# Dxslab/mpi-petsc4py-example

Measured on AMD Instinct MI355X. Metric: CG iters/s + SpMV HBM GB/s (% peak), 3D Poisson 256³ at 1/2/4/8 GPUs, higher is better.
Workload: dtype f64

## Files before the change

mpi-petsc4py-example_amd/csrc/mx_abi.hip:

```cpp
#include <algorithm>
#include <atomic>
#include <cmath>
#include <cstdio>
#include <cstring>
#include <mutex>
#include <string>
#include <thread>
#include <vector>

#include "mx_internal.hpp"

struct mx_comm_s { mx::Comm *c; };
struct mx_mat_s { mx::Mat *A; };

namespace mx {

static thread_local std::string g_err;

[[noreturn]] void fail(int code, const std::string &msg) { throw Error(code, msg); }

void hip_check(hipError_t e, const char *what, const char *file, int line) {
  if (e != hipSuccess) {
    char buf[512];
    std::snprintf(buf, sizeof buf, "%s failed: %s (%s:%d)", what, hipGetErrorString(e), file, line);
// ... 550 lines not shown
  });
}
int mx_ksp_destroy(mx_mat a) {
  return guard([&] {
    Mat *A = M(a);
    (void)hipSetDevice(A->comm->device);
    HIPCHECK(hipStreamSynchronize(A->comm->stream));
    A->release_ksp();
  });
}
int mx_finalize(void) {
  return guard([&] {
    int nd = 0;
    if (hipGetDeviceCount(&nd) != hipSuccess) nd = 0;
    for (int d = 0; d < nd; ++d) {
      if (hipSetDevice(d) == hipSuccess) HIPCHECK(hipDeviceSynchronize());
    }
    (void)hipGetLastError();
    scratch_trim();
  });
}
int mx_vec_rhs_hash(mx_comm c, int64_t i0, int64_t n, double *b) {
  return guard([&] { Comm *k = C(c); vec_rhs_hash(k->stream, i0, n, b); HIPCHECK(hipStreamSynchronize(k->stream)); });
}

void mx_ksp_default_params(mx_ksp_params *p) {
  std::memset(p, 0, sizeof(*p));
  p->ksp_type = MX_KSP_GMRES;
  p->pc_type = MX_PC_JACOBI;
  p->norm_type = MX_NORM_DEFAULT;
  p->max_it = 10000;
  p->restart = 30;
  p->rtol = 1e-5;
  p->atol = 1e-50;
  p->dtol = 1e5;
  p->haptol = 1e-30;
  p->breakdowntol = 0.1;
  p->poll_every = 16;
}

int mx_lu_solve_csr(mx_comm c, int64_t n, const int64_t *indptr, const int64_t *cols,
                    const double *vals, const double *b, double *x) {
  return guard([&] { dense_lu_solve(C(c), n, indptr, cols, vals, b, x); });
}

int mx_dev_alloc(int device, size_t bytes, void **ptr) {
  return guard([&] {
    HIPCHECK(hipSetDevice(device));
    *ptr = nullptr;
    if (bytes && dev_malloc(ptr, bytes) != hipSuccess) { *ptr = nullptr; fail(MX_ERR_MEM, "device allocation failed"); }
  });
}

int mx_dev_free(void *ptr) { return guard([&] { dev_free(ptr); }); }

int mx_debug_set(int key, int value) {
  int old = -1;
  switch (key) {
    case 6: old = g_knobs.overlap; g_knobs.overlap = value; break;
    case 7: old = g_knobs.graph; g_knobs.graph = value; break;
    case 8: old = g_knobs.force_coll; g_knobs.force_coll = value; break;
    case 9: old = g_knobs.cg_fuse; g_knobs.cg_fuse = value; break;
    case 13: old = g_knobs.cg_vec; g_knobs.cg_vec = value; break;
    case 21: old = g_knobs.cg_unroll; g_knobs.cg_unroll = value; break;
    case 23: old = g_knobs.vcodes; g_knobs.vcodes = value; break;
    case 27: old = g_knobs.spmv_pairs; g_knobs.spmv_pairs = value; break;
    case 29: old = g_knobs.cg_xbatch; g_knobs.cg_xbatch = value; break;
    case 33: old = g_knobs.comm_timeout_ms; if (value > 0) g_knobs.comm_timeout_ms = value; break;
    case 38: old = g_knobs.pair_lean; g_knobs.pair_lean = value; break;
    case 39: old = g_knobs.pair_zm; g_knobs.pair_zm = value; break;
    case 40: old = g_knobs.pair_zm_bpc; g_knobs.pair_zm_bpc = std::min(std::max(value, 1), 8); break;
    case 41: old = g_knobs.pair_zm_len; g_knobs.pair_zm_len = std::min(std::max(value, 1), 1024); break;
    case 43: old = g_knobs.spmv_fp64_grid; g_knobs.spmv_fp64_grid = std::min(std::max(value, 0), 65536); break;
    case 47: old = g_knobs.comm_wait_ms; g_knobs.comm_wait_ms = std::max(value, 0); break;
    case 48: old = g_knobs.pair_col27; g_knobs.pair_col27 = value; break;
    case 52: old = g_knobs.pair_zmc; g_knobs.pair_zmc = value; break;
    case 53: old = g_knobs.pair_unitv; g_knobs.pair_unitv = value; break;
    case 60: old = g_knobs.pair_zm27p; g_knobs.pair_zm27p = value; break;
    case 70: old = g_knobs.zm27_2line; g_knobs.zm27_2line = value; break;
    case 72: old = g_knobs.asm_fused; g_knobs.asm_fused = value; break;
    case 80: old = g_knobs.cg_pbws; g_knobs.cg_pbws = value; break;
    case 81: old = g_knobs.scratch_cache; g_knobs.scratch_cache = value; if (!value) scratch_trim(); break;
    case 84: old = g_knobs.cb; g_knobs.cb = value; break;
    case 69: old = g_knobs.cg_pbw; g_knobs.cg_pbw = value; break;
    case 68: old = g_knobs.ru_2line; g_knobs.ru_2line = value; break;
    case 61: old = g_knobs.gm_stall_us; g_knobs.gm_stall_us = std::min(std::max(value, 0), 2000000); break;
    case 59: old = g_knobs.pw_sym27; g_knobs.pw_sym27 = value; break;
    default: break;
  }
  return old;
}

int mx_debug_assembly_times(double *out, int n) {
  const AsmTimes &t = g_asm_times;
  const double v[8] = {t.h2d_ms, t.canon_ms, t.split_ms, t.layout_ms, t.halo_ms, t.total_ms, t.host_bytes, t.alloc_ms};
  for (int k = 0; k < n && k < 8; ++k) out[k] = v[k];
  return 0;
}

int mx_debug_dispatch_counts(int64_t *out, int n, int reset) {
  for (int k = 0; k < DSP_COUNT; ++k) {
    const long long v = reset ? g_dispatch[k].exchange(0) : g_dispatch[k].load();
    if (out && k < n) out[k] = v;
  }
  return 0;
}

int mx_debug_stream_read(mx_comm c, const double *x, int64_t n, int width, double *out) {
  return guard([&] {
    Comm *k = C(c);
    debug_stream_read(k->stream, x, n, width, out);
    HIPCHECK(hipStreamSynchronize(k->stream));
  });
}

int mx_ksp_solve(mx_mat a, const mx_ksp_params *p, const double *b, double *x, mx_ksp_result *res,
                 double *history) {
  return guard([&] {
    Mat *A = M(a);
    ksp_solve(A, *p, b, x, *res, history);
  });
}

}

namespace mx {
void h2d_warm() {
  constexpr size_t W = (size_t)32 << 20;
  char *h = static_cast<char *>(std::aligned_alloc(4096, W));
  void *d = nullptr;
  hipStream_t st = nullptr;
  if (h && hipMalloc(&d, W) == hipSuccess && hipStreamCreateWithFlags(&st, hipStreamNonBlocking) == hipSuccess) {
    std::memset(h, 0, W);
    try {
      h2d_pinned({{d, h, W}}, st, (size_t)1 << 20);
    } catch (const Error &) {
    }
  }
  if (st) (void)hipStreamDestroy(st);
  if (d) (void)hipFree(d);
  std::free(h);
  (void)hipGetLastError();
}
}
```

mpi-petsc4py-example_amd/csrc/mx_internal.hpp:

```cpp
#pragma once

#include <hip/hip_runtime.h>

#include <atomic>
#include <cstdint>
#include <functional>
#include <memory>
#include <stdexcept>
#include <string>
#include <vector>

#include "mxsolve.h"

namespace mx {

struct Error : std::runtime_error {
  int code;
  Error(int c, const std::string &m) : std::runtime_error(m), code(c) {}
};

[[noreturn]] void fail(int code, const std::string &msg);
void hip_check(hipError_t e, const char *what, const char *file, int line);
#define HIPCHECK(x) ::mx::hip_check((x), #x, __FILE__, __LINE__)

// ... 78 lines not shown
  uint32_t lane[64];
};
struct PairUni27 {
  double v[54];
  unsigned long long pm[54];
  uint32_t flags, clean;
  uint32_t pad[2];
  unsigned long long lane[64];
};
constexpr uint32_t U27_ELO = 1u << 9;
constexpr uint32_t U27_EHI = 1u << 10;
constexpr uint32_t U27C_YLO = 1u << 0;
constexpr uint32_t U27C_YHI = 1u << 1;

struct Sell {
  int64_t nslices = 0, slots = 0, dia_slices = 0;
  int dia_k = 0;
  DBuf<int64_t> sptr;
  DBuf<int32_t> width;
  DBuf<int32_t> col;
  DBuf<double> val;
  DBuf<int32_t> doff;
  DBuf<int32_t> dpat;
  int64_t npat = 0;
  DBuf<uint32_t> mask;
  DBuf<uint8_t> mask8;
  int ntab = 0;
  int64_t code_bytes = 0;
  DBuf<uint8_t> code;
  DBuf<int64_t> cptr;
  DBuf<double> vtab;
  int32_t pat_star = -1;
  std::vector<int32_t> pat_star_off;
  std::vector<int32_t> pat_len;
  std::vector<int32_t> pat_host;
  int pair_shape = 0;
  int64_t nunits = 0;
  DBuf<uint8_t> pcode;
  DBuf<int32_t> pblk;
  int64_t pair_blocks = 0;
  int64_t pair_used = 0;
  bool pair_ghosts = false;
  bool pair_all = false;
  DBuf<PairUni> puni;
  bool pair_clean = false;
  DBuf<PairUni27> puni27;
  DBuf<double> pval;
  DBuf<int32_t> pflag;
  int pair_f64 = 0;
  bool pair_clean27 = false;
  bool pair_unit27 = false;
  bool pair_sym27 = false;
  bool pair_2l27 = false;
  bool pair_4l27 = false;
  DBuf<int32_t> pcol27;
  DBuf<double> dtab;
  bool pair_code_clean = false;
  int cb_bs = 0, cb_nblk = 0;
  DBuf<int64_t> cb_bstart;
  DBuf<int32_t> cb_col, cb_perm;
  DBuf<double> cb_val, cb_prod;
};
constexpr uint32_t PBLK_GHOST_LO = 1u << 30;
constexpr uint32_t PBLK_GHOST_HI = 1u << 31;
constexpr uint32_t PBLK_RUN0 = 1u << 22;
constexpr uint32_t PBLK_ELO = 1u << 27;
constexpr uint32_t PBLK_EHI = 1u << 28;
constexpr uint32_t PBLK_ID = PBLK_RUN0 - 1;
static_assert((PBLK_RUN0 << 4) < PBLK_ELO && PBLK_ELO < PBLK_EHI && PBLK_EHI < PBLK_GHOST_LO,
              "PBLK select-free flags overlap the ghost bits");
static_assert(((PBLK_RUN0 << 5) - PBLK_RUN0 | PBLK_ELO | PBLK_EHI | PBLK_ID) < PBLK_GHOST_LO, "PBLK field overlap");
constexpr int64_t PAIR_MAX_ROWS = int64_t(1) << 28;
constexpr int VCODE_MAX = 256;
constexpr int VCODE_ABSENT = VCODE_MAX - 1;
constexpr int CODE_BATCH = 8 * SLICE;
struct VCodes { const uint8_t *code; const int64_t *cptr; const double *tab; int ntab; };

struct Knobs {
  int overlap = 1; int graph = 1; int force_coll = 0; int cg_fuse = 3; int cg_vec = 0; int cg_unroll = 2;
  int vcodes = 1; int spmv_pairs = 1; int cg_xbatch = 0; int comm_timeout_ms = 120000;
  int pair_lean = 1; int pair_zm = 1; int pair_zm_bpc = 4; int pair_zm_len = 32; int spmv_fp64_grid = 8192;
  int comm_wait_ms = 600000; int pair_col27 = 1; int pair_zmc = 1; int pair_unitv = 1; int pw_sym27 = 1;
  int pair_zm27p = 1; int gm_stall_us = 0; int ru_2line = 3; int cg_pbw = 5; int zm27_2line = 1;
  int asm_fused = 1; int cg_pbws = 1; int scratch_cache = 1; int cb = 1;
  static constexpr int spmv_nt = 1, spmv_grid = 0, dia = 1, jac_const = 1, cg_fold = 1, ws_skew = 0;
  static constexpr int cg_vec_grid = 0, cg_nts = 0, bnd_grid = 0, mask8 = 1, cg_upd_grid = 0, spmv_ynt = 0;
  static constexpr int spmv_bpc = 6, spmv_pair_bpc = 4, pdict = 1, cg_ntl = 3, norm_grid = 0, pair_uni = 1;
  static constexpr int mdot_grid = 0, pair_dtab = 1, pair_zm_units = 2, pair_f64 = 1, pair_zm27_bpc = 6;
  static constexpr int cg5_fold = 1, pair_zm27_units = 1, gm_pad = 256, cg5_27 = 1, pair_zm27_ru_bpc = 5;
  static constexpr int pw_bpc = 0, ru_bpc = 3, zm_balance = 1, zm27_xcol = 1, zm27_xcol_ru = 2, zm27_xcol_pw = 3;
  static constexpr int maxpy_grid = 0, zmc_units = 1, zmc_bpc = 0;
};
extern Knobs g_knobs;

struct Halo {
  std::vector<int> recv_peer;
  std::vector<int64_t> recv_off, recv_cnt;
  std::vector<int> send_peer;
  std::vector<int64_t> send_off, send_cnt;
  std::vector<int64_t> send_contig_start;
  DBuf<int32_t> send_idx;
  DBuf<double> send_buf;
  DBuf<double> lvec;
  int64_t nsend = 0, nrecv = 0;
  bool need_pack = false;
  DBuf<int32_t> bnd_slices;
  int nbnd = 0;
  hipEvent_t ev_x = nullptr, ev_done = nullptr;
  ~Halo() {
    if (ev_x) (void)hipEventDestroy(ev_x);
    if (ev_done) (void)hipEventDestroy(ev_done);
  }
};

struct Mat {
  Comm *comm = nullptr;
  int64_t M = 0, N = 0, m = 0, n = 0, rstart = 0, cstart = 0, cend = 0;
  std::vector<int64_t> rranges, cranges;
  DBuf<int64_t> dptr, optr;
  DBuf<int32_t> dcol, ocol;
  DBuf<double> dval, oval, diag;
  DBuf<int64_t> garray;
  int64_t nnz_d = 0, nnz_o = 0, nghost = 0;
  std::vector<int64_t> garray_h;
  Sell sd, so;
  Halo halo;
  DBuf<double> partials;
  DBuf<double> scratch_x;
  DBuf<double> ksp_ws;
  DBuf<char> ksp_state;
  DBuf<double> jac_dinv;
  int jac_mode = -1;
  double jac_c = 1.0;
  int sym = -1;
  hipGraphExec_t cg_graph = nullptr;
  std::vector<uintptr_t> cg_key;
  bool cg_graph_failed = false;
  int *poll_pinned = nullptr;
  void *state_pinned = nullptr;
  hipEvent_t poll_ev[2] = {nullptr, nullptr};
  hipEvent_t solve_ev[2] = {nullptr, nullptr};
  void release_ksp();
  ~Mat() { release_ksp(); }
};

struct AsmTimes {
  double h2d_ms = 0, canon_ms = 0, split_ms = 0, layout_ms = 0, halo_ms = 0, total_ms = 0;
  double alloc_ms = 0;
  double host_bytes = 0;
};
extern thread_local AsmTimes g_asm_times;
double wall_ms();

struct AssemblyInput {
  const int64_t *rowptr = nullptr;
  const int64_t *coo_rows = nullptr;
  const int64_t *cols = nullptr;
  const int32_t *cols32 = nullptr;
  const double *vals = nullptr;
  int64_t nnz = 0;
  int insert_mode = MX_INSERT_VALUES;
};
Mat *assemble(Comm *c, int64_t M, int64_t N, int64_t m_local, int64_t n_local,
              const AssemblyInput &in);
void stencil_coo(Comm *c, int kind, int64_t nx, int64_t ny, int64_t nz, int64_t row0,
                 int64_t m, DBuf<int64_t> &rows, DBuf<int64_t> &cols, DBuf<int32_t> &cols32,
                 DBuf<double> &vals);
void convert_index(const void *src, int bytes, int64_t n, int64_t *dst, hipStream_t s);

struct Jac {
  const double *d = nullptr;
  double c = 1.0;
  int mode = 0;
};
__device__ __forceinline__ double papply(const Jac &J, double r, int64_t i) {
  return J.mode == 1 ? r * J.d[i] : (J.mode == 2 ? r * J.c : r);
}

enum SpmvMode { SPMV_PLAIN = 0, SPMV_JACOBI = 1, SPMV_DOT = 2, SPMV_CG = 3,
                SPMV_PLAIN_S = 4, SPMV_JACOBI_S = 5,
                SPMV_PW = 6, SPMV_RUPD = 7 };
constexpr bool spmv_jac(int mode) { return mode == SPMV_JACOBI || mode == SPMV_JACOBI_S; }
constexpr bool spmv_scaled(int mode) { return mode == SPMV_PLAIN_S || mode == SPMV_JACOBI_S; }
struct KspState;
struct Fold;
struct CgFuse {
  const double *r = nullptr;
  const double *pold = nullptr;
  double *pnew = nullptr;
  double *x = nullptr;
  KspState *st = nullptr;
  double *hist = nullptr;
  Jac jac;
};
void halo_begin(Mat *A, const double *x);
void spmv_launch(Mat *A, const double *x, double *y, int mode, Jac jac, double *partials,
                 int *done_flag);
int matmult_overlap(Mat *A, const double *x, double *y, int mode, Jac jac, double *partials,
                    int *done_flag, const CgFuse *cg = nullptr, const Fold *fold = nullptr,
                    const double *xscale = nullptr);
int spmv_blocks(const Mat *A, int mode = SPMV_PLAIN);
struct ExtTiming { hipEvent_t a = nullptr, b = nullptr; bool armed = false, used = false; };
extern thread_local ExtTiming g_ext_timing;
enum Dispatch {
  DSP_SELL = 0,
  DSP_SELL_CG = 1,
  DSP_PAIR_LEAN = 2,
  DSP_PAIR_ZM = 3,
  DSP_PAIR_ZM_SPLIT = 4,
  DSP_PAIR_ZM27 = 5,
  DSP_PAIR_ZM27_SPLIT = 6,
  DSP_PAIR_ZMF64 = 7,
  DSP_PAIR_ZMF64_SPLIT = 8,
  DSP_PAIR_ZMCG = 9,
  DSP_BOUNDARY = 10,
  DSP_ZM_PW = 11,
  DSP_ZM_RUPD = 12,
  DSP_PAIR_ZMC = 13,
  DSP_PAIR_ZMC_SPLIT = 14,
  DSP_ZM_PBW = 15,
  DSP_ZM_PBWS = 16,
  DSP_CB = 17,
  DSP_COUNT = 18
};
void note_dispatch(int kind);
extern std::atomic<long long> g_dispatch[DSP_COUNT];
int device_cu_count();
int main_grid(const Mat *A, int mode, const void *kf, bool pairs);
int pair_lean_launch(Mat *A, int mode, bool split, const double *x, double *y, double *partials, const int *done,
                     const Fold &fold, hipStream_t st, const Jac &jac = Jac{}, const double *xscale = nullptr);
bool pair_code_applies(const Mat *A);
void pair_sym_prepare(Mat *A);
int pair_lean_kind(const Mat *A);
bool pair_zm_applies(const Mat *A);
int pair_f64_kind(const Mat *A);
bool pair_cg5_applies(const Mat *A, int jac_mode);
int pair_cg5_rupd_launch(Mat *A, KspState *s, const double *p, const double *w, double *r, const double *r0,
                         int jac_mode, double jac_c, double *partials, const Fold &fold, const double *dot_part,
                         int ndot, int xb, int *hw, hipStream_t st);
bool pair_cg5_pbw_applies(const Mat *A, int jac_mode, int xb);
int pair_cg5_pbw_launch(Mat *A, KspState *s, const double *r, const double *r0, double *const pb[8], int xb,
                        double *hist, int jac_mode, double jac_c, double *partials, const Fold &fold,
                        hipStream_t st);
bool pair_cg5_pbws_applies(const Mat *A, int jac_mode, int xb);
int pair_cg5_pbws_launch(Mat *A, KspState *s, const double *r, double *const pb[8], int xb, double *hist, int jac_mode,
                         double jac_c, double *y, double *partials, hipStream_t st);
int cg5_pbws_matmult(Mat *A, KspState *s, const double *r, double *const pb[8], int xb, int it, double *hist,
                     const Jac &jac, double *y, double *partials, int *done, const Fold *fold);
bool matmult_splits(const Mat *A);
void mat_mult(Mat *A, const double *x, double *y);
void build_cb(Mat *A, hipStream_t st);
bool cb_applies(const Mat *A, int mode, bool split);
int cb_launch(Mat *A, int mode, bool split, const double *x, double *y, const Jac &jac, double *partials,
              const int *done, const Fold &fold, const double *xscale, hipStream_t st);

constexpr int RED_BLOCKS = 1024;
void finish_reduce(const double *partials, int nblocks, int nvals, double *out, hipStream_t s,
                   int *done_flag = nullptr);
double host_dot(Comm *c, int64_t n, const double *x, const double *y);
void host_mdot(Comm *c, int64_t n, const double *x, int nv, const double *const *y, double *out_host);
void vec_maxpy(hipStream_t s, int64_t n, double *y, int nv, const double *alpha, const double *const *x);
void vec_axpy(hipStream_t s, int64_t n, double a, const double *x, double *y);
void vec_aypx(hipStream_t s, int64_t n, double a, const double *x, double *y);
void vec_pmult(hipStream_t s, int64_t n, const double *x, const double *y, double *w);
void vec_scale(hipStream_t s, int64_t n, double a, double *x);
void vec_set(hipStream_t s, int64_t n, double a, double *x);
void vec_rhs_hash(hipStream_t s, int64_t i0, int64_t n, double *b);
void debug_stall(hipStream_t s, int stall_us);
void flush_read(hipStream_t s, const double *x, int64_t n, double *partials);
void debug_stream_read(hipStream_t s, const double *x, int64_t n, int width, double *out);
void exclusive_scan_i64(const int64_t *in, int64_t *out, int64_t n, hipStream_t s,
                        int64_t *total_host);

void dense_lu_solve(Comm *c, int64_t n, const int64_t *ip, const int64_t *cj, const double *vv,
                    const double *b, double *x);

void ksp_solve(Mat *A, const mx_ksp_params &p, const double *b, double *x, mx_ksp_result &r,
               double *hist);

inline int64_t cdiv(int64_t a, int64_t b) { return (a + b - 1) / b; }
inline unsigned grid_for(int64_t n, int block, int64_t cap = 1 << 16) {
  int64_t g = cdiv(n, block);
  if (g < 1) g = 1;
  if (g > cap) g = cap;
  return (unsigned)g;
}

void load_code_comm();
void load_code_vec();
void load_code_assembly();
void load_code_spmv();
void load_code_spmv_pair();
void load_code_spmv_cb();
void load_code_ksp();
void load_code_direct();
void load_code_objects();
void h2d_warm();

}
```

mpi-petsc4py-example_amd/csrc/mx_spmv_pair.hip:

```cpp
#include "mx_cg.hpp"
#include "mx_device.hpp"
#include "mx_internal.hpp"
#include "mx_pair.hpp"
#include "mx_launch.hpp"

namespace mx {

constexpr int PAIR_OOR = 1 << 28;
constexpr int PAIR_OOR_EDGE = 1 << 27;
constexpr int64_t PAIR_CLEAN_MAX_ROWS = int64_t(1) << 27;
constexpr int LEAN_WAVES = 4;

struct PairLeanArgs {
  int m, n, nunits;
  int anchor[5];
  int P, NZ, L, S;
  double *partials;
  const int *done;
  Fold fold;
};

template <int PS, bool CLEAN>
__device__ __forceinline__ dbl2 pair_sums(const dbl2 (&L)[PairShape<PS>::NR], double e, uint32_t bw,
                                          const PairUni *__restrict__ puni, int lane) {
// ... 280 lines not shown
  int sb, se, W, w;
  if ((gridDim.x & 7) == 0) {
    const int xcd = blockIdx.x & 7;
    W = (gridDim.x >> 3) * LEAN_WAVES;
    w = (blockIdx.x >> 3) * LEAN_WAVES + wid;
    sb = a.S * xcd / 8;
    se = a.S * (xcd + 1) / 8;
  } else {
    W = gridDim.x * LEAN_WAVES;
    w = blockIdx.x * LEAN_WAVES + wid;
    sb = 0;
    se = a.S;
  }
  const __amdgpu_buffer_rsrc_t xr = vec_rsrc(x, a.n);
  const int D = a.anchor[LAST], NL = a.anchor[3];
  const int PL = NL / 128, PH = a.P / 2;
  const int ecst = lane == 0 ? a.anchor[TR] - 1 : 128 + a.anchor[TR];
  constexpr uint32_t CARRY = PBLK_RUN0 | (PBLK_RUN0 << TR) | (PBLK_RUN0 << LAST);
  double nv[3] = {0.0, 0.0, 0.0};
  const int ntask = (se - sb) * PH;
  for (int t = w; t < ntask; t += W) {
    const int seg = sb + t / PH, cp = t % PH;
    const int colA = (cp / PL) * 2 * PL + cp % PL, colB = colA + PL;
    const int z0 = seg * a.L, z1 = min(z0 + a.L, a.NZ);
    const int cbA = colA * 128 + 2 * lane, cbB = colB * 128 + 2 * lane;
    dbl2 zmA = bload2(xr, z0 * D + cbA - D), cA = bload2(xr, z0 * D + cbA);
    dbl2 zmB = bload2(xr, z0 * D + cbB - D), cB = bload2(xr, z0 * D + cbB);
    uint32_t bwAn = (uint32_t)pblk[z0 * a.P + colA], bwBn = (uint32_t)pblk[z0 * a.P + colB];
    for (int z = z0; z < z1; ++z) {
      const uint32_t bwA = bwAn, bwB = bwBn;
      if (z + 1 < z1) { bwAn = (uint32_t)pblk[(z + 1) * a.P + colA]; bwBn = (uint32_t)pblk[(z + 1) * a.P + colB]; }
      const int rA = z * D + cbA, rB = z * D + cbB;
      const dbl2 zpA = bload2(xr, rA + D), zpB = bload2(xr, rB + D);
      const dbl2 nA = bload2(xr, rA + a.anchor[1] + ((bwA & (PBLK_RUN0 << 1)) ? PAIR_OOR : 0));
      const dbl2 nB = bload2(xr, rB + a.anchor[3] + ((bwB & (PBLK_RUN0 << 3)) ? PAIR_OOR : 0));
      int eA = ecst, eB = ecst;
      eA += lane == 0 ? ((bwA & PBLK_ELO) ? PAIR_OOR : 0) : ((bwA & PBLK_EHI) ? PAIR_OOR : 0);
      eB += lane == 0 ? ((bwB & PBLK_ELO) ? PAIR_OOR : 0) : ((bwB & PBLK_EHI) ? PAIR_OOR : 0);
      const double edA = bload1(xr, z * D + colA * 128 + eA), edB = bload1(xr, z * D + colB * 128 + eB);
      const dbl2 rqA = __builtin_nontemporal_load(reinterpret_cast<const dbl2 *>(rin + rA));
      const dbl2 rqB = __builtin_nontemporal_load(reinterpret_cast<const dbl2 *>(rin + rB));
      __builtin_amdgcn_sched_barrier(0);
      const dbl2 Z{0.0, 0.0};
      dbl2 LA[NR] = {zmA, nA, cA, (bwA & (PBLK_RUN0 << 3)) ? Z : cB, zpA};
      dbl2 LB[NR] = {zmB, (bwB & (PBLK_RUN0 << 1)) ? Z : cA, cB, nB, zpB};
      if (bwA & CARRY) {
        if (bwA & PBLK_RUN0) LA[0] = Z;
        if (bwA & (PBLK_RUN0 << TR)) LA[TR] = Z;
        if (bwA & (PBLK_RUN0 << LAST)) LA[LAST] = Z;
      }
      if (bwB & CARRY) {
        if (bwB & PBLK_RUN0) LB[0] = Z;
        if (bwB & (PBLK_RUN0 << TR)) LB[TR] = Z;
        if (bwB & (PBLK_RUN0 << LAST)) LB[LAST] = Z;
      }
      const dbl2 wA = pair_sums<PS, true>(LA, edA, bwA, puni, lane);
      const dbl2 wB = pair_sums<PS, true>(LB, edB, bwB, puni, lane);
      auto upd = [&](dbl2 w2, dbl2 rq, int r0) __attribute__((always_inline)) {
        const double ra = fma(-alpha, w2.x, rq.x), rb = fma(-alpha, w2.y, rq.y);
        const double za = JM == 2 ? ra * ru.c : ra, zb = JM == 2 ? rb * ru.c : rb;
        nv[0] += za * za; nv[1] += za * ra; nv[2] += ra * ra;
        nv[0] += zb * zb; nv[1] += zb * rb; nv[2] += rb * rb;
        *reinterpret_cast<dbl2 *>(ru.r + r0) = dbl2{ra, rb};
      };
      upd(wA, rqA, rA);
      upd(wB, rqB, rB);
      zmA = cA; cA = zpA;
      zmB = cB; cB = zpB;
    }
  }
  block_partials<3>(nv, a.partials, gridDim.x, a.fold);
}

struct PairPbArgs {
  KspState *s;
  const double *r;
  const double *r0;
  double *pb;
  int64_t ps;
  double *hist;
  double c;
};

template <int PS, int JM, int B, int ZU>
__global__ void __launch_bounds__(256) spmv_pair_pbw_kernel(const PairLeanArgs a, const int32_t *__restrict__ pblk,
                                                            const PairUni *__restrict__ puni, const PairPbArgs pa) {
  KspState *s = pa.s;
  const CgTopIn top = s->top;
  if (top.done) return;
  const CgTop t = cg_top(top);
  if (blockIdx.x == 0 && threadIdx.x == 0) cg_commit_top(s, t, pa.hist);
  if (t.reason) return;
  const int i = t.i;
  const double b = t.b;
  using SH = PairShape<PS>;
  constexpr int NR = SH::NR, TR = PS == 5 ? 1 : 2, LAST = NR - 1, C = SH::CENTER_RUN;
  auto pick = [&](int k) -> double * { return pa.pb + k * pa.ps; };
  double *pout = pick(i % B);
  const double *pprev = pick((i + B - 1) % B);
  const double *rs = (pa.r0 && i == 0) ? pa.r0 : pa.r;
  const int lane = threadIdx.x & 63;
  const int wid = __builtin_amdgcn_readfirstlane(threadIdx.x >> 6);
  int sb, se, W, w;
  if ((gridDim.x & 7) == 0) {
    const int xcd = blockIdx.x & 7;
    W = (gridDim.x >> 3) * LEAN_WAVES;
    w = (blockIdx.x >> 3) * LEAN_WAVES + wid;
    sb = a.S * xcd / 8;
    se = a.S * (xcd + 1) / 8;
  } else {
    W = gridDim.x * LEAN_WAVES;
    w = blockIdx.x * LEAN_WAVES + wid;
    sb = 0;
    se = a.S;
  }
  const __amdgpu_buffer_rsrc_t rr = vec_rsrc(rs, a.n), pr = vec_rsrc(pprev, a.n);
  const int D = a.anchor[LAST];
  const int eoff = 128 + a.anchor[TR];
  constexpr uint32_t CARRY = PBLK_RUN0 | (PBLK_RUN0 << TR) | (PBLK_RUN0 << LAST);
  const int ntask = (se - sb) * a.P;
  double dot = 0.0;
  auto march = [&](auto npc) __attribute__((always_inline)) {
    constexpr bool NP = decltype(npc)::value;
    auto dir = [&](dbl2 r2, dbl2 p2) __attribute__((always_inline)) {
      return dbl2{cg_dir(jac1<JM>(r2.x, 0.0, pa.c), b, NP ? 0.0 : p2.x),
                  cg_dir(jac1<JM>(r2.y, 0.0, pa.c), b, NP ? 0.0 : p2.y)};
    };
    for (int tk = w; tk < ntask; tk += W) {
      const int seg = sb + tk / a.P, col = tk % a.P;
      const int z0 = seg * a.L, z1 = min(z0 + a.L, a.NZ);
      const int cb = col * 128 + 2 * lane;
      dbl2 pc = dir(bload2(rr, z0 * D + cb), NP ? dbl2{0.0, 0.0} : bload2(pr, z0 * D + cb));
      uint32_t bwn = (uint32_t)pblk[z0 * a.P + col];
      auto step = [&](int z, auto nq) __attribute__((always_inline)) {
        constexpr int NQ = decltype(nq)::value;
        dbl2 zr[NQ], zpp[NQ], nr[NQ], npp[NQ];
        double er[NQ], epp[NQ];
        uint32_t bw[NQ];
        bw[0] = bwn;
#pragma unroll
        for (int q = 1; q < NQ; ++q) bw[q] = (uint32_t)pblk[(z + q) * a.P + col];
        if (z + NQ < z1) bwn = (uint32_t)pblk[(z + NQ) * a.P + col];
#pragma unroll
        for (int q = 0; q < NQ; ++q) {
          const int r0 = (z + q) * D + cb, ub = (z + q) * D + col * 128;
          zr[q] = bload2(rr, r0 + D);
          zpp[q] = NP ? dbl2{0.0, 0.0} : bload2(pr, r0 + D);
          if constexpr (PS == 7) {
            const int no = r0 + a.anchor[3] + ((bw[q] & (PBLK_RUN0 << 3)) ? PAIR_OOR : 0);
            nr[q] = bload2(rr, no);
            npp[q] = NP ? dbl2{0.0, 0.0} : bload2(pr, no);
          }
          er[q] = 0.0;
          epp[q] = 0.0;
          if (!(bw[q] & PBLK_EHI)) {
            er[q] = bload1(rr, ub + eoff);
            if constexpr (!NP) epp[q] = bload1(pr, ub + eoff);
          }
        }
        __builtin_amdgcn_sched_barrier(0);
#pragma unroll
        for (int q = 0; q < NQ; ++q) {
          const int r0 = (z + q) * D + cb;
          const dbl2 pz = dir(zr[q], zpp[q]);
          const double pe = cg_dir(jac1<JM>(er[q], 0.0, pa.c), b, NP ? 0.0 : epp[q]);
          *reinterpret_cast<dbl2 *>(pout + r0) = pc;
          dbl2 L[NR];
          L[0] = dbl2{0.0, 0.0};
          if constexpr (PS == 7) { L[1] = dbl2{0.0, 0.0}; L[3] = dir(nr[q], npp[q]); }
          L[TR] = pc;
          L[LAST] = pz;
          if (bw[q] & CARRY) {
            if (bw[q] & (PBLK_RUN0 << TR)) L[TR] = dbl2{0.0, 0.0};
            if (bw[q] & (PBLK_RUN0 << LAST)) L[LAST] = dbl2{0.0, 0.0};
          }
          const dbl2 tq = pair_fwd<PS>(L, pe, bw[q], puni);
          dot += L[C].x * tq.x;
          dot += L[C].y * tq.y;
          pc = pz;
        }
      };
      int z = z0;
      for (; z + ZU <= z1; z += ZU) step(z, std::integral_constant<int, ZU>{});
      for (; z < z1; ++z) step(z, std::integral_constant<int, 1>{});
    }
  };
  const std::true_type T{};
  const std::false_type F{};
  if (b == 0.0) march(T);
  else march(F);
  double v[1] = {dot};
  block_partials<1>(v, a.partials, gridDim.x, a.fold);
}

template <int PS, bool CLEAN, int ZU, int JM>
__global__ void __launch_bounds__(256) spmv_pair_zmpbs_kernel(const PairLeanArgs a, double *__restrict__ y,
                                                              const int32_t *__restrict__ pblk,
                                                              const PairUni *__restrict__ puni, const PairPbArgs pa,
                                                              int xb) {
  KspState *s = pa.s;
  const CgTopIn top = s->top;
  if (top.done) return;
  const CgTop t = cg_top(top);
  if (blockIdx.x == 0 && threadIdx.x == 0) cg_commit_top(s, t, pa.hist);
  if (t.reason) return;
  const int i = t.i;
  const double b = t.b;
  double *pout = pa.pb + (int64_t)(i % xb) * pa.ps;
  const double *pprev = pa.pb + (int64_t)((i + xb - 1) % xb) * pa.ps;
  using SH = PairShape<PS>;
  constexpr int NR = SH::NR, TR = PS == 5 ? 1 : 2, LAST = NR - 1;
  const int lane = threadIdx.x & 63;
  const int wid = __builtin_amdgcn_readfirstlane(threadIdx.x >> 6);
  int sb, se, W, w;
  if ((gridDim.x & 7) == 0) {
    const int xcd = blockIdx.x & 7;
    W = (gridDim.x >> 3) * LEAN_WAVES;
    w = (blockIdx.x >> 3) * LEAN_WAVES + wid;
    sb = a.S * xcd / 8;
    se = a.S * (xcd + 1) / 8;
  } else {
    W = gridDim.x * LEAN_WAVES;
    w = blockIdx.x * LEAN_WAVES + wid;
    sb = 0;
    se = a.S;
  }
  const __amdgpu_buffer_rsrc_t rr = vec_rsrc(pa.r, a.n), pr = vec_rsrc(pprev, a.n);
  const int D = a.anchor[LAST];
  const int ecst = lane == 0 ? a.anchor[TR] - 1 : 128 + a.anchor[TR];
  constexpr uint32_t CARRY = PBLK_RUN0 | (PBLK_RUN0 << TR) | (PBLK_RUN0 << LAST);
  auto dir1 = [&](double r1, double p1) __attribute__((always_inline)) {
    return cg_dir(jac1<JM>(r1, 0.0, pa.c), b, p1);
  };
  auto dir2 = [&](dbl2 r2, dbl2 p2) __attribute__((always_inline)) { return dbl2{dir1(r2.x, p2.x), dir1(r2.y, p2.y)}; };
  auto ld2 = [&](int off) __attribute__((always_inline)) { return dir2(bload2(rr, off), bload2(pr, off)); };
  double dot = 0.0;
  const int ntask = (se - sb) * a.P;
  for (int tk = w; tk < ntask; tk += W) {
    const int seg = sb + tk / a.P, col = tk % a.P;
    const int z0 = seg * a.L, z1 = min(z0 + a.L, a.NZ);
    const int cb = col * 128 + 2 * lane;
    dbl2 zm = ld2(z0 * D + cb - D), c = ld2(z0 * D + cb);
    uint32_t bwn = (uint32_t)pblk[z0 * a.P + col];
    auto step = [&](int z, auto nq) __attribute__((always_inline)) {
      constexpr int NQ = decltype(nq)::value;
      dbl2 L[NQ][NR], zp[NQ], zr[NQ], zq[NQ], Lr[NQ][NR], Lp[NQ][NR];
      double e[NQ], er[NQ], ep[NQ];
      uint32_t bw[NQ];
      bw[0] = bwn;
#pragma unroll
      for (int q = 1; q < NQ; ++q) bw[q] = (uint32_t)pblk[(z + q) * a.P + col];
      if (z + NQ < z1) bwn = (uint32_t)pblk[(z + NQ) * a.P + col];
#pragma unroll
      for (int q = 0; q < NQ; ++q) {
        const int r0 = (z + q) * D + cb, ub = (z + q) * D + col * 128;
        zr[q] = bload2(rr, r0 + D);
        zq[q] = bload2(pr, r0 + D);
#pragma unroll
        for (int r = 1; r < LAST; ++r)
          if (r != TR) {
            const int off = r0 + a.anchor[r] + (CLEAN && (bw[q] & (PBLK_RUN0 << r)) ? PAIR_OOR : 0);
            Lr[q][r] = bload2(rr, off);
            Lp[q][r] = bload2(pr, off);
          }
        int eo = ecst;
        if constexpr (CLEAN) eo += lane == 0 ? ((bw[q] & PBLK_ELO) ? PAIR_OOR : 0) : ((bw[q] & PBLK_EHI) ? PAIR_OOR : 0);
        er[q] = bload1(rr, ub + eo);
        ep[q] = bload1(pr, ub + eo);
      }
      __builtin_amdgcn_sched_barrier(0);
#pragma unroll
      for (int q = 0; q < NQ; ++q) {
// ... 1262 lines not shown
  if (pair_code_applies(A) && (split || (A->nghost == 0 && !S.pair_ghosts)))
    return pair_code_launch(A, mode, split, x, y, partials, done, fold_in, jac, xscale, st);
  if (xscale) return 0;
  if (mode != SPMV_PLAIN && mode != SPMV_DOT && mode != SPMV_PW) return 0;
  if (mode == SPMV_PW && !pair_cg5_applies(A, 0)) return 0;
  if (pair_f64_kind(A) && (split || A->nghost == 0))
    return pair_f64_launch(A, mode, split, x, y, partials, done, fold_in, st);
  const int kind = pair_lean_kind(A);
  if (!kind) return 0;
  if (!split && (A->nghost > 0 || S.pair_ghosts)) return 0;
  const bool clean = kind == 2;
  if (S.pair_shape == 27) return zm27_launch(A, mode, split, clean, x, y, partials, done, fold_in, st, PairRuArgs{}, 0);
  PairLeanArgs a{};
  a.m = (int)A->m;
  a.n = (int)A->n;
  a.nunits = (int)S.nunits;
  pair_anchors(S, a.anchor);
  a.partials = partials;
  a.done = done;
  const int NR = S.pair_shape == 5 ? 3 : 5, D = a.anchor[NR - 1];
  const bool zm = pair_zm_applies(A);
  LeanFn f = nullptr;
  ZmFn fz = nullptr;
  int grid;
  if (zm) {
    a.P = D / 128;
    a.NZ = (int)(A->m / D);
    grid = zm_tasks(a.P, a.NZ, a.L, a.S, mode == SPMV_PW && g_knobs.pw_bpc > 0 ? g_knobs.pw_bpc : g_knobs.pair_zm_bpc);
#define ZM_PICK(MODE, PS, SP, CL) \
    fz = g_knobs.pair_zm_units == 2 ? &spmv_pair_zm_kernel<MODE, PS, SP, CL, 2> : &spmv_pair_zm_kernel<MODE, PS, SP, CL, 1>
#define ZM_C(MODE, PS) do { if (split) { if (clean) ZM_PICK(MODE, PS, true, true); else ZM_PICK(MODE, PS, true, false); } \
                            else { if (clean) ZM_PICK(MODE, PS, false, true); else ZM_PICK(MODE, PS, false, false); } } while (0)
    if (mode == SPMV_PLAIN) { if (S.pair_shape == 5) ZM_C(SPMV_PLAIN, 5); else ZM_C(SPMV_PLAIN, 7); }
    else if (mode == SPMV_PW && clean && !split && A->sym == 1 && g_knobs.pw_sym27) {
      if (S.pair_shape == 5) fz = g_knobs.pair_zm_units == 2 ? &spmv_pair_zm_kernel<SPMV_PW, 5, false, true, 2, 0, true>
                                                             : &spmv_pair_zm_kernel<SPMV_PW, 5, false, true, 1, 0, true>;
      else fz = g_knobs.pair_zm_units == 2 ? &spmv_pair_zm_kernel<SPMV_PW, 7, false, true, 2, 0, true>
                                           : &spmv_pair_zm_kernel<SPMV_PW, 7, false, true, 1, 0, true>;
    }
    else if (mode == SPMV_PW) { if (S.pair_shape == 5) ZM_C(SPMV_PW, 5); else ZM_C(SPMV_PW, 7); }
    else { if (S.pair_shape == 5) ZM_C(SPMV_DOT, 5); else ZM_C(SPMV_DOT, 7); }
#undef ZM_C
#undef ZM_PICK
  } else {
#define LEAN_C(MODE, PS) do { if (split) f = clean ? &spmv_pair_lean_kernel<MODE, PS, true, true> : &spmv_pair_lean_kernel<MODE, PS, true, false>; \
                              else f = clean ? &spmv_pair_lean_kernel<MODE, PS, false, true> : &spmv_pair_lean_kernel<MODE, PS, false, false>; } while (0)
    if (mode == SPMV_PLAIN) { if (S.pair_shape == 5) LEAN_C(SPMV_PLAIN, 5); else LEAN_C(SPMV_PLAIN, 7); }
    else { if (S.pair_shape == 5) LEAN_C(SPMV_DOT, 5); else LEAN_C(SPMV_DOT, 7); }
#undef LEAN_C
    grid = main_grid(A, mode, reinterpret_cast<const void *>(f), true);
  }
  Fold fold = fold_in;
  if (fold.cnt) { fold.ntotal = fold.ncount = grid; fold.base = 0; }
  a.fold = fold;
  note_dispatch(mode == SPMV_PW ? DSP_ZM_PW : !zm ? DSP_PAIR_LEAN : split ? DSP_PAIR_ZM_SPLIT : DSP_PAIR_ZM);
  if (zm) launch_timed(fz, grid, st, a, x, y, S.pblk.p, S.puni.p, PairRuArgs{});
  else launch_timed(f, grid, st, a, x, y, S.pblk.p, S.puni.p);
  HIPCHECK(hipGetLastError());
  return grid;
}

bool pair_cg5_applies(const Mat *A, int jac_mode) {
  if (jac_mode != 0 && jac_mode != 2) return false;
  if (A->sd.pair_shape == 27)
    return g_knobs.cg5_27 && pair_lean_kind(A) == 2 && A->sd.pcol27.p && A->nghost == 0 && !A->sd.pair_ghosts;
  return pair_lean_kind(A) > 0 && pair_zm_applies(A) && ((A->nghost == 0 && !A->sd.pair_ghosts) || matmult_splits(A));
}

static int cg5_args(const Mat *A, PairLeanArgs &a, int bpc = 0) {
  const Sell &S = A->sd;
  a = PairLeanArgs{};
  a.m = (int)A->m;
  a.n = (int)A->n;
  a.nunits = (int)S.nunits;
  pair_anchors(S, a.anchor);
  const int D = a.anchor[S.pair_shape == 5 ? 2 : 4];
  a.P = D / 128;
  a.NZ = (int)(A->m / D);
  return zm_tasks(a.P, a.NZ, a.L, a.S, bpc);
}

bool pair_cg5_pbw_applies(const Mat *A, int jac_mode, int xb) {
  const int on = g_knobs.cg_pbw != 5 ? g_knobs.cg_pbw
                                     : A->m <= (int64_t(1) << (A->sd.pair_shape == 5 ? 24 : 23));
  return on && (xb == 2 || xb == 4 || xb == 8) && (jac_mode == 0 || jac_mode == 2) && pair_cg5_applies(A, jac_mode) &&
         A->sd.pair_shape != 27 && pair_lean_kind(A) == 2 && A->nghost == 0 && !A->sd.pair_ghosts && A->sym == 1 &&
         g_knobs.pw_sym27 && pair_zm_applies(A);
}

int pair_cg5_pbw_launch(Mat *A, KspState *s, const double *r, const double *r0, double *const pb[8], int xb,
                        double *hist, int jac_mode, double jac_c, double *partials, const Fold &fold_in,
                        hipStream_t st) {
  if (!pair_cg5_pbw_applies(A, jac_mode, xb)) return 0;
  const Sell &S = A->sd;
  PairLeanArgs a{};
  a.m = (int)A->m;
  a.n = (int)A->n;
  a.nunits = (int)S.nunits;
  pair_anchors(S, a.anchor);
  a.partials = partials;
  const int NR = S.pair_shape == 5 ? 3 : 5, D = a.anchor[NR - 1];
  a.P = D / 128;
  a.NZ = (int)(A->m / D);
  const int grid = zm_tasks(a.P, a.NZ, a.L, a.S, g_knobs.pw_bpc > 0 ? g_knobs.pw_bpc : g_knobs.pair_zm_bpc);
  Fold fold = fold_in;
  if (fold.cnt) { fold.ntotal = fold.ncount = grid; fold.base = 0; }
  a.fold = fold;
  const PairPbArgs pa{s, r, r0, pb[0], pb[1] - pb[0], hist, jac_c};
  using PbwFn = void (*)(const PairLeanArgs, const int32_t *, const PairUni *, const PairPbArgs);
  PbwFn f;
  const bool z2 = g_knobs.pair_zm_units == 2;
#define PBW(PS, JM, B) f = z2 ? &spmv_pair_pbw_kernel<PS, JM, B, 2> : &spmv_pair_pbw_kernel<PS, JM, B, 1>
#define PBW_B(PS, JM) do { if (xb == 8) PBW(PS, JM, 8); else if (xb == 4) PBW(PS, JM, 4); else PBW(PS, JM, 2); } while (0)
#define PBW_J(PS) do { if (jac_mode == 2) PBW_B(PS, 2); else PBW_B(PS, 0); } while (0)
  if (S.pair_shape == 5) PBW_J(5);
  else PBW_J(7);
#undef PBW_J
#undef PBW_B
#undef PBW
  note_dispatch(DSP_ZM_PBW);
  launch_timed(f, grid, st, a, S.pblk.p, S.puni.p, pa);
  HIPCHECK(hipGetLastError());
  return grid;
}

bool pair_cg5_pbws_applies(const Mat *A, int jac_mode, int xb) {
  return g_knobs.cg_pbws && A->comm->size > 1 && (xb == 2 || xb == 4 || xb == 8) &&
         (jac_mode == 0 || jac_mode == 2) && A->sd.pair_shape != 27 && pair_cg5_applies(A, jac_mode) &&
         matmult_splits(A) && pair_lean_kind(A) > 0 && pair_zm_applies(A);
}

int pair_cg5_pbws_launch(Mat *A, KspState *s, const double *r, double *const pb[8], int xb, double *hist, int jac_mode,
                         double jac_c, double *y, double *partials, hipStream_t st) {
  const Sell &S = A->sd;
  PairLeanArgs a{};
  a.m = (int)A->m;
  a.n = (int)A->n;
  a.nunits = (int)S.nunits;
  pair_anchors(S, a.anchor);
  a.partials = partials;
  const int NR = S.pair_shape == 5 ? 3 : 5, D = a.anchor[NR - 1];
  a.P = D / 128;
  a.NZ = (int)(A->m / D);
  const int grid = zm_tasks(a.P, a.NZ, a.L, a.S, g_knobs.pw_bpc > 0 ? g_knobs.pw_bpc : g_knobs.pair_zm_bpc);
  a.fold = Fold{};
  const PairPbArgs pa{s, r, nullptr, pb[0], pb[1] - pb[0], hist, jac_c};
  using Fn = void (*)(const PairLeanArgs, double *, const int32_t *, const PairUni *, const PairPbArgs, int);
  Fn f;
  const bool clean = pair_lean_kind(A) == 2, z2 = g_knobs.pair_zm_units == 2;
#define PBS(PS, CL, JM) f = z2 ? &spmv_pair_zmpbs_kernel<PS, CL, 2, JM> : &spmv_pair_zmpbs_kernel<PS, CL, 1, JM>
#define PBS_J(PS, CL) do { if (jac_mode == 2) PBS(PS, CL, 2); else PBS(PS, CL, 0); } while (0)
#define PBS_C(PS) do { if (clean) PBS_J(PS, true); else PBS_J(PS, false); } while (0)
  if (S.pair_shape == 5) PBS_C(5);
  else PBS_C(7);
#undef PBS_C
#undef PBS_J
#undef PBS
  note_dispatch(DSP_ZM_PBWS);
  launch_timed(f, grid, st, a, y, S.pblk.p, S.puni.p, pa, xb);
  HIPCHECK(hipGetLastError());
  return grid;
}

int pair_cg5_rupd_launch(Mat *A, KspState *s, const double *p, const double *w, double *r, const double *r0,
                         int jac_mode, double jac_c, double *partials, const Fold &fold_in, const double *dot_part,
                         int ndot, int xb, int *hw, hipStream_t st) {
  if (!pair_cg5_applies(A, jac_mode)) return 0;
  if (A->sd.pair_shape == 27) {
    const PairRuArgs ru{s, w, r, r0, dot_part, ndot, xb, jac_c, hw};
    return zm27_launch(A, SPMV_RUPD, false, true, p, nullptr, partials, nullptr, fold_in, st, ru, jac_mode);
  }
  PairLeanArgs a;
  const int grid = cg5_args(A, a, g_knobs.ru_bpc);
  a.partials = partials;
  Fold fold = fold_in;
  if (fold.cnt) { fold.ntotal = fold.ncount = grid; fold.base = 0; }
  a.fold = fold;
  const bool split = A->sd.pair_ghosts;
  const PairRuArgs ru{s, w, r, r0, dot_part, ndot, xb, jac_c, hw};
  const bool clean = pair_lean_kind(A) == 2, z2 = g_knobs.pair_zm_units == 2;
  ZmFn f;
#define RU(PS, SP, CL, JM) f = z2 ? &spmv_pair_zm_kernel<SPMV_RUPD, PS, SP, CL, 2, JM> \
                                  : &spmv_pair_zm_kernel<SPMV_RUPD, PS, SP, CL, 1, JM>
#define RU_S(PS, CL, JM) do { if (split) RU(PS, true, CL, JM); else RU(PS, false, CL, JM); } while (0)
#define RU_J(PS, CL) do { if (jac_mode == 2) RU_S(PS, CL, 2); else RU_S(PS, CL, 0); } while (0)
  if (A->sd.pair_shape == 5) { if (clean) RU_J(5, true); else RU_J(5, false); }
  else { if (clean) RU_J(7, true); else RU_J(7, false); }
#undef RU_J
#undef RU_S
#undef RU
  const int two = g_knobs.ru_2line == 3 ? (A->m >= (int64_t(1) << 23) ? 2 : 0) : g_knobs.ru_2line;
  if (two && clean && !split && A->sd.pair_shape == 7 && a.anchor[3] > 0 && a.anchor[3] % 128 == 0 &&
      (a.anchor[4] / a.anchor[3]) % 2 == 0 && a.anchor[4] % a.anchor[3] == 0 && a.anchor[1] == -a.anchor[3]) {
    int L2, S2;
    const int g2 = zm_tasks(a.P / 2, a.NZ, L2, S2, g_knobs.ru_bpc);
    a.L = L2;
    a.S = S2;
    if (fold.cnt) { fold.ntotal = fold.ncount = g2; fold.base = 0; }
    a.fold = fold;
    note_dispatch(DSP_ZM_RUPD);
    const bool w5 = two == 2;
    if (jac_mode == 2) launch_timed(w5 ? &spmv_pair_zm2l_kernel<2, 5> : &spmv_pair_zm2l_kernel<2, 1>, g2, st, a, p,
// ... 20 lines not shown
```

mpi-petsc4py-example_amd/mxsolve/core.py:

```python
from __future__ import annotations

import ctypes as C
import os
import threading

import numpy as np
import torch

from . import _lib
from ._lib import KSPParams, KSPResult, MatInfo, MxError, call

KSP_TYPES = {"cg": 0, "gmres": 1, "preonly": 2}
PC_TYPES = {"none": 0, "jacobi": 1}
NORM_TYPES = {"default": -1, "none": 0, "preconditioned": 1, "unpreconditioned": 2, "natural": 3}
STENCILS = {"poisson2d": 0, "poisson3d": 1, "poisson3d27": 2, "convdiff3d": 3}


def _ptr(t) -> C.c_void_p:
    if isinstance(t, torch.Tensor):
        if not t.is_cuda or t.dtype != torch.float64 or not t.is_contiguous():
            raise TypeError("device vectors must be contiguous float64 CUDA tensors")
        return C.c_void_p(t.data_ptr())
    if t is None:
        return C.c_void_p(0)
# ... 269 lines not shown

    def solve(self, b: torch.Tensor, x: torch.Tensor, ksp: str = "cg", pc: str = "jacobi",
              rtol: float = 1e-5, atol: float = 1e-50, dtol: float = 1e5, max_it: int = 10000,
              restart: int = 30, norm: str = "default", guess_nonzero: bool = False,
              history: bool = False, profile: bool = False, poll_every: int = 16) -> dict:
        p = KSPParams()
        _lib.load().mx_ksp_default_params(C.byref(p))
        p.ksp_type, p.pc_type, p.norm_type = KSP_TYPES[ksp], PC_TYPES[pc], NORM_TYPES[norm]
        p.rtol, p.atol, p.dtol, p.max_it, p.restart = rtol, atol, dtol, max_it, restart
        p.guess_nonzero, p.profile, p.poll_every = int(guess_nonzero), int(profile), poll_every
        r = KSPResult()
        h = np.zeros(max_it + 2) if history else None
        call("mx_ksp_solve", self.h, C.byref(p), _ptr(b), _ptr(x), C.byref(r),
             C.c_void_p(h.ctypes.data) if history else C.c_void_p(0))
        out = {k: getattr(r, k) for k, _ in KSPResult._fields_}
        if history:
            out["history"] = h[: r.its + 1]
        return out

    def ksp_reset(self):
        if self.h and self.comm.h:
            call("mx_ksp_destroy", self.h)

    def destroy(self):
        if self.h:
            if self.comm.h:
                call("mx_mat_destroy", self.h)
            self.h = None

    def __del__(self):
        try:
            self.destroy()
        except Exception:
            pass


def vdot(comm: DeviceComm, x, y) -> float:
    out = C.c_double()
    call("mx_vec_dot", comm.h, x.numel(), _ptr(x), _ptr(y), C.byref(out))
    return out.value


def vnorm(comm: DeviceComm, x) -> float:
    out = C.c_double()
    call("mx_vec_norm2", comm.h, x.numel(), _ptr(x), C.byref(out))
    return out.value


def vaxpy(comm, a, x, y):
    call("mx_vec_axpy", comm.h, y.numel(), float(a), _ptr(x), _ptr(y))


def vaypx(comm, a, x, y):
    call("mx_vec_aypx", comm.h, y.numel(), float(a), _ptr(x), _ptr(y))


def vpmult(comm, x, y, w):
    call("mx_vec_pointwise_mult", comm.h, w.numel(), _ptr(x), _ptr(y), _ptr(w))


def vscale(comm, a, x):
    call("mx_vec_scale", comm.h, x.numel(), float(a), _ptr(x))


def vset(comm, a, x):
    call("mx_vec_set", comm.h, x.numel(), float(a), _ptr(x))


def vmdot(comm: DeviceComm, x, ys) -> np.ndarray:
    arr = (C.c_void_p * max(len(ys), 1))(*[_ptr(y).value for y in ys])
    out = np.zeros(len(ys))
    call("mx_vec_mdot", comm.h, x.numel(), _ptr(x), len(ys), arr, out.ctypes.data_as(C.POINTER(C.c_double)))
    return out


def vmaxpy(comm: DeviceComm, y, alphas, xs):
    arr = (C.c_void_p * max(len(xs), 1))(*[_ptr(v).value for v in xs])
    a = np.ascontiguousarray(alphas, dtype=np.float64)
    call("mx_vec_maxpy", comm.h, y.numel(), _ptr(y), len(xs), a.ctypes.data_as(C.POINTER(C.c_double)), arr)


DISPATCH_KINDS = ("sell", "sell_cg", "pair_lean", "pair_zm", "pair_zm_split", "pair_zm27", "pair_zm27_split",
                  "pair_zmf64", "pair_zmf64_split", "pair_zmcg", "boundary", "zm_pw", "zm_rupd", "pair_zmc",
                  "pair_zmc_split", "zm_pbw", "zm_pbws", "cb")


def dispatch_counts(reset: bool = False) -> dict:
    out = (C.c_int64 * len(DISPATCH_KINDS))()
    call("mx_debug_dispatch_counts", out, len(DISPATCH_KINDS), int(reset))
    return {k: int(out[i]) for i, k in enumerate(DISPATCH_KINDS)}


ASM_PHASES = ("h2d_ms", "canon_ms", "split_ms", "layout_ms", "halo_ms", "total_ms", "host_bytes", "alloc_ms")


def assembly_times() -> dict:
    out = (C.c_double * len(ASM_PHASES))()
    call("mx_debug_assembly_times", out, len(ASM_PHASES))
    return {k: float(out[i]) for i, k in enumerate(ASM_PHASES)}


def rhs_hash(comm, i0: int, out: torch.Tensor):
    call("mx_vec_rhs_hash", comm.h, i0, out.numel(), _ptr(out))
```

Before: 5649.

## Share neighbor-row direction values through LDS in 7-point fused CG pbw kernel

Adds a shared-memory variant of the fused p-update/SpMV kernel for 7-point stencils. Waves write their freshly computed direction values into a double-buffered LDS exchange array, so neighbors along y and x read them from LDS instead of reloading and recomputing them from global r/p. It also widens the size threshold for the pbw path on 7-point matrices so it covers larger local problems. The cost is a __syncthreads per z step plus register pinning via inline asm, and the variant only applies under layout divisibility conditions.

New measurement: 5771, median of 6. +2.2%, better.

```diff
diff --git a/mpi-petsc4py-example_amd/csrc/mx_abi.hip b/mpi-petsc4py-example_amd/csrc/mx_abi.hip
--- a/mpi-petsc4py-example_amd/csrc/mx_abi.hip
+++ b/mpi-petsc4py-example_amd/csrc/mx_abi.hip
@@ -656,6 +656,7 @@
     case 80: old = g_knobs.cg_pbws; g_knobs.cg_pbws = value; break;
     case 81: old = g_knobs.scratch_cache; g_knobs.scratch_cache = value; if (!value) scratch_trim(); break;
     case 84: old = g_knobs.cb; g_knobs.cb = value; break;
+    case 85: old = g_knobs.zm_shared; g_knobs.zm_shared = value; break;
     case 69: old = g_knobs.cg_pbw; g_knobs.cg_pbw = value; break;
     case 68: old = g_knobs.ru_2line; g_knobs.ru_2line = value; break;
     case 61: old = g_knobs.gm_stall_us; g_knobs.gm_stall_us = std::min(std::max(value, 0), 2000000); break;
diff --git a/mpi-petsc4py-example_amd/csrc/mx_internal.hpp b/mpi-petsc4py-example_amd/csrc/mx_internal.hpp
--- a/mpi-petsc4py-example_amd/csrc/mx_internal.hpp
+++ b/mpi-petsc4py-example_amd/csrc/mx_internal.hpp
@@ -184,7 +184,7 @@
   int pair_lean = 1; int pair_zm = 1; int pair_zm_bpc = 4; int pair_zm_len = 32; int spmv_fp64_grid = 8192;
   int comm_wait_ms = 600000; int pair_col27 = 1; int pair_zmc = 1; int pair_unitv = 1; int pw_sym27 = 1;
   int pair_zm27p = 1; int gm_stall_us = 0; int ru_2line = 3; int cg_pbw = 5; int zm27_2line = 1;
-  int asm_fused = 1; int cg_pbws = 1; int scratch_cache = 1; int cb = 1;
+  int asm_fused = 1; int cg_pbws = 1; int scratch_cache = 1; int cb = 1; int zm_shared = 1;
   static constexpr int spmv_nt = 1, spmv_grid = 0, dia = 1, jac_const = 1, cg_fold = 1, ws_skew = 0;
   static constexpr int cg_vec_grid = 0, cg_nts = 0, bnd_grid = 0, mask8 = 1, cg_upd_grid = 0, spmv_ynt = 0;
   static constexpr int spmv_bpc = 6, spmv_pair_bpc = 4, pdict = 1, cg_ntl = 3, norm_grid = 0, pair_uni = 1;
@@ -323,7 +323,8 @@
   DSP_ZM_PBW = 15,
   DSP_ZM_PBWS = 16,
   DSP_CB = 17,
-  DSP_COUNT = 18
+  DSP_ZM_SHARED = 18,
+  DSP_COUNT = 19
 };
 void note_dispatch(int kind);
 extern std::atomic<long long> g_dispatch[DSP_COUNT];
diff --git a/mpi-petsc4py-example_amd/csrc/mx_spmv_pair.hip b/mpi-petsc4py-example_amd/csrc/mx_spmv_pair.hip
--- a/mpi-petsc4py-example_amd/csrc/mx_spmv_pair.hip
+++ b/mpi-petsc4py-example_amd/csrc/mx_spmv_pair.hip
@@ -386,7 +386,7 @@
   double c;
 };
 
-template <int PS, int JM, int B, int ZU>
+template <int PS, int JM, int B, int ZU, bool XS = false>
 __global__ void __launch_bounds__(256) spmv_pair_pbw_kernel(const PairLeanArgs a, const int32_t *__restrict__ pblk,
                                                             const PairUni *__restrict__ puni, const PairPbArgs pa) {
   KspState *s = pa.s;
@@ -396,7 +396,7 @@
   if (blockIdx.x == 0 && threadIdx.x == 0) cg_commit_top(s, t, pa.hist);
   if (t.reason) return;
   const int i = t.i;
-  const double b = t.b;
+  double b = t.b;
   using SH = PairShape<PS>;
   constexpr int NR = SH::NR, TR = PS == 5 ? 1 : 2, LAST = NR - 1, C = SH::CENTER_RUN;
   auto pick = [&](int k) -> double * { return pa.pb + k * pa.ps; };
@@ -419,21 +419,33 @@
     se = a.S;
   }
   const __amdgpu_buffer_rsrc_t rr = vec_rsrc(rs, a.n), pr = vec_rsrc(pprev, a.n);
-  const int D = a.anchor[LAST];
-  const int eoff = 128 + a.anchor[TR];
+  int D = a.anchor[LAST];
+  int eoff = 128 + a.anchor[TR];
+  double jc = pa.c;
+  if constexpr (XS) {
+    asm volatile("" : "+v"(b), "+v"(jc), "+v"(D), "+v"(eoff));
+  }
   constexpr uint32_t CARRY = PBLK_RUN0 | (PBLK_RUN0 << TR) | (PBLK_RUN0 << LAST);
   const int ntask = (se - sb) * a.P;
   double dot = 0.0;
+  static_assert(!XS || PS == 7, "shared form: 7-point");
+  __shared__ dbl2 xch[XS ? 2 * LEAN_WAVES * 64 : 1];
+  const int PL = XS ? a.anchor[3] / 128 : 1;
+  int xw = wid * 64 + lane, xn = xw + PL * 64, xe = xw + 1;
   auto march = [&](auto npc) __attribute__((always_inline)) {
     constexpr bool NP = decltype(npc)::value;
     auto dir = [&](dbl2 r2, dbl2 p2) __attribute__((always_inline)) {
-      return dbl2{cg_dir(jac1<JM>(r2.x, 0.0, pa.c), b, NP ? 0.0 : p2.x),
-                  cg_dir(jac1<JM>(r2.y, 0.0, pa.c), b, NP ? 0.0 : p2.y)};
+      return dbl2{cg_dir(jac1<JM>(r2.x, 0.0, jc), b, NP ? 0.0 : p2.x),
+                  cg_dir(jac1<JM>(r2.y, 0.0, jc), b, NP ? 0.0 : p2.y)};
     };
-    for (int tk = w; tk < ntask; tk += W) {
+    for (int tb = w - wid; tb < ntask; tb += W) {
+      const int tk = tb + wid;
+      if constexpr (!XS) { if (tk >= ntask) break; }
       const int seg = sb + tk / a.P, col = tk % a.P;
       const int z0 = seg * a.L, z1 = min(z0 + a.L, a.NZ);
       const int cb = col * 128 + 2 * lane;
+      const bool dnIn = XS && PL < 4 && wid + PL < LEAN_WAVES;
+      const bool hiIn = XS && wid < LEAN_WAVES - 1 && col % PL < PL - 1;
       dbl2 pc = dir(bload2(rr, z0 * D + cb), NP ? dbl2{0.0, 0.0} : bload2(pr, z0 * D + cb));
       uint32_t bwn = (uint32_t)pblk[z0 * a.P + col];
       auto step = [&](int z, auto nq) __attribute__((always_inline)) {
@@ -445,19 +457,24 @@
 #pragma unroll
         for (int q = 1; q < NQ; ++q) bw[q] = (uint32_t)pblk[(z + q) * a.P + col];
         if (z + NQ < z1) bwn = (uint32_t)pblk[(z + NQ) * a.P + col];
+        if constexpr (XS) xch[xw] = pc;
 #pragma unroll
         for (int q = 0; q < NQ; ++q) {
           const int r0 = (z + q) * D + cb, ub = (z + q) * D + col * 128;
           zr[q] = bload2(rr, r0 + D);
           zpp[q] = NP ? dbl2{0.0, 0.0} : bload2(pr, r0 + D);
           if constexpr (PS == 7) {
-            const int no = r0 + a.anchor[3] + ((bw[q] & (PBLK_RUN0 << 3)) ? PAIR_OOR : 0);
-            nr[q] = bload2(rr, no);
-            npp[q] = NP ? dbl2{0.0, 0.0} : bload2(pr, no);
+            nr[q] = dbl2{0.0, 0.0};
+            npp[q] = dbl2{0.0, 0.0};
+            if (!dnIn) {
+              const int no = r0 + a.anchor[3] + ((bw[q] & (PBLK_RUN0 << 3)) ? PAIR_OOR : 0);
+              nr[q] = bload2(rr, no);
+              npp[q] = NP ? dbl2{0.0, 0.0} : bload2(pr, no);
+            }
           }
           er[q] = 0.0;
           epp[q] = 0.0;
-          if (!(bw[q] & PBLK_EHI)) {
+          if (!(bw[q] & PBLK_EHI) && !hiIn) {
             er[q] = bload1(rr, ub + eoff);
             if constexpr (!NP) epp[q] = bload1(pr, ub + eoff);
           }
@@ -467,11 +484,18 @@
         for (int q = 0; q < NQ; ++q) {
           const int r0 = (z + q) * D + cb;
           const dbl2 pz = dir(zr[q], zpp[q]);
-          const double pe = cg_dir(jac1<JM>(er[q], 0.0, pa.c), b, NP ? 0.0 : epp[q]);
+          double pe = cg_dir(jac1<JM>(er[q], 0.0, jc), b, NP ? 0.0 : epp[q]);
           *reinterpret_cast<dbl2 *>(pout + r0) = pc;
           dbl2 L[NR];
           L[0] = dbl2{0.0, 0.0};
           if constexpr (PS == 7) { L[1] = dbl2{0.0, 0.0}; L[3] = dir(nr[q], npp[q]); }
+          if constexpr (XS && PS == 7) {
+            if (q > 0) xch[xw] = pc;
+            __syncthreads();
+            if (dnIn) L[3] = (bw[q] & (PBLK_RUN0 << 3)) ? dbl2{0.0, 0.0} : xch[xn];
+            if (hiIn && !(bw[q] & PBLK_EHI) && lane == 63) pe = xch[xe].x;
+            xw ^= LEAN_WAVES * 64; xn ^= LEAN_WAVES * 64; xe ^= LEAN_WAVES * 64;
+          }
           L[TR] = pc;
           L[LAST] = pz;
           if (bw[q] & CARRY) {
@@ -491,7 +515,7 @@
   };
   const std::true_type T{};
   const std::false_type F{};
-  if (b == 0.0) march(T);
+  if (t.b == 0.0) march(T);
   else march(F);
   double v[1] = {dot};
   block_partials<1>(v, a.partials, gridDim.x, a.fold);
@@ -1920,7 +1944,7 @@
 
 bool pair_cg5_pbw_applies(const Mat *A, int jac_mode, int xb) {
   const int on = g_knobs.cg_pbw != 5 ? g_knobs.cg_pbw
-                                     : A->m <= (int64_t(1) << (A->sd.pair_shape == 5 ? 24 : 23));
+                                     : A->m <= (int64_t(1) << 24);
   return on && (xb == 2 || xb == 4 || xb == 8) && (jac_mode == 0 || jac_mode == 2) && pair_cg5_applies(A, jac_mode) &&
          A->sd.pair_shape != 27 && pair_lean_kind(A) == 2 && A->nghost == 0 && !A->sd.pair_ghosts && A->sym == 1 &&
          g_knobs.pw_sym27 && pair_zm_applies(A);
@@ -1956,6 +1980,17 @@
 #undef PBW_J
 #undef PBW_B
 #undef PBW
+  const int NL = S.pair_shape == 7 ? a.anchor[3] : 0, PL = NL / 128;
+  if (g_knobs.zm_shared && z2 && NL > 0 && NL % 128 == 0 && D % NL == 0 && a.P % 4 == 0 &&
+      (PL == 1 || PL == 2 || PL % 4 == 0) && grid % 8 == 0) {
+#define PBWS(JM) do { if (xb == 8) f = &spmv_pair_pbw_kernel<7, JM, 8, 2, true>; \
+                      else if (xb == 4) f = &spmv_pair_pbw_kernel<7, JM, 4, 2, true>; \
+                      else f = &spmv_pair_pbw_kernel<7, JM, 2, 2, true>; } while (0)
+    if (jac_mode == 2) PBWS(2);
+    else PBWS(0);
+#undef PBWS
+    note_dispatch(DSP_ZM_SHARED);
+  }
   note_dispatch(DSP_ZM_PBW);
   launch_timed(f, grid, st, a, S.pblk.p, S.puni.p, pa);
   HIPCHECK(hipGetLastError());
diff --git a/mpi-petsc4py-example_amd/mxsolve/core.py b/mpi-petsc4py-example_amd/mxsolve/core.py
--- a/mpi-petsc4py-example_amd/mxsolve/core.py
+++ b/mpi-petsc4py-example_amd/mxsolve/core.py
@@ -375,7 +375,7 @@
 
 DISPATCH_KINDS = ("sell", "sell_cg", "pair_lean", "pair_zm", "pair_zm_split", "pair_zm27", "pair_zm27_split",
                   "pair_zmf64", "pair_zmf64_split", "pair_zmcg", "boundary", "zm_pw", "zm_rupd", "pair_zmc",
-                  "pair_zmc_split", "zm_pbw", "zm_pbws", "cb")
+                  "pair_zmc_split", "zm_pbw", "zm_pbws", "cb", "zm_shared")
 
 
 def dispatch_counts(reset: bool = False) -> dict:
```
